# atsuki-ichikawa/KoeMorph

Hardware: AMD Instinct MI355X
Metric: blendshape frames/sec (52-coef, 256-win, d_model=256) (higher is better)
Workload: dtype f32; 1 GPU; C2: 256 windows/GPU x 136448 samples (8.5 s @16 kHz) -> 1024-pt STFT, hop 533, 80-bin log-mel (257 frames) -> dual-stream attention d_model=256, 8 heads, window 256 -> 52 coefficients + EMA; from audio resident in HBM (rotating batches); windows_per_gpu=256, samples_per_window=136448, parallelism=window-sharded x1, no collective

## Files before the change

### include/koemorph.h

```cpp
#ifndef KOEMORPH_H
#define KOEMORPH_H

#include <stdint.h>

#ifdef __cplusplus
extern "C" {
#endif

#define KM_ABI_VERSION 2

typedef enum km_status {
    KM_OK = 0,
    KM_ERR_INVALID_ARG = -1,
    KM_ERR_UNSUPPORTED = -2,
    KM_ERR_NOT_FINALIZED = -3,
    KM_ERR_WORKSPACE = -4,
    KM_ERR_HIP = -5,
    KM_ERR_NOT_READY = -6
} km_status;

typedef struct km_context* km_handle;

typedef enum km_mel_scale { KM_MEL_SLANEY = 0, KM_MEL_HTK = 1 } km_mel_scale;
typedef enum km_pad_mode { KM_PAD_CONSTANT = 0, KM_PAD_REFLECT = 1 } km_pad_mode;
// ... 228 lines not shown
                        void* stream);
int km_stream_step_attn(km_handle h, const float* emotion_dev, float* out_dev, uint8_t* fired_dev, uint8_t* ready_dev, int32_t* backlog_dev,
                        float* raw_dev, float* attn_dev, void* stream);

int km_legacy_stream_create(km_handle h, int64_t n_streams, int64_t buffer_samples, int64_t audio_length);
int km_legacy_stream_push(km_handle h, const float* samples_dev, int64_t n_per_stream, const int32_t* counts_dev, void* stream);
int km_legacy_stream_tick(km_handle h, float* out_dev, uint8_t* ready_dev, void* stream);
int km_legacy_stream_reset(km_handle h, void* stream);

int km_enable_stage_timing(km_handle h, int32_t enable);
int km_stage_times(km_handle h, float* ms3);

int km_egemaps_plan_create(void** plan_out);
int km_egemaps_plan_destroy(void* plan);
int64_t km_egemaps_num_frames(int64_t L);
int64_t km_egemaps_workspace_floats(int64_t B, int64_t L);
int km_egemaps_functionals(void* plan, const float* audio_dev, int64_t B, int64_t L, int32_t normalize, float* work_dev,
                           int64_t work_floats, float* out_dev, void* stream);
int km_egemaps_records(const float* work_dev, int64_t B, int64_t L, float* rec_host, void* stream);
int km_egemaps_track_from_records(float* rec_dev, int64_t B, int64_t nf, void* stream);
int km_egemaps_functionals_from_records(const float* rec_dev, int64_t B, int64_t nf, float* out_dev, void* stream);
int km_linear(const float* x_dev, const float* w_dev, const float* b_dev, int64_t B, int64_t K, int64_t N, float* out_dev, void* stream);
int km_gemm_kernel_choice(int64_t M, int64_t N, int64_t K, int64_t batch);

int km_emotion_stream_create(void** es, int64_t n_streams, double context_window_s, double update_interval_s, int64_t max_updates);
int km_emotion_stream_destroy(void* es);
int km_emotion_stream_set_compression(void* es, const float* w_dev, const float* b_dev, void* stream);
int km_emotion_stream_push(void* es, const float* samples_dev, int64_t n_per_stream, const int32_t* counts_dev, void* stream);
int km_emotion_stream_update(void* es, float* emotion_dev, uint8_t* valid_dev, uint8_t* updated_dev, void* stream);
int km_emotion_stream_reset_streams(void* es, const uint8_t* mask_dev, void* stream);
int km_emotion_stream_features(void* es, float* features_dev, float* slots_dev, void* stream);

int km_prosody_plan_create(void** plan_out);
int km_prosody_plan_destroy(void* plan);
int64_t km_prosody_num_frames(int64_t L);
int64_t km_prosody_workspace_floats(int64_t B, int64_t L);
int km_prosody_features(void* plan, const float* audio_dev, int64_t B, int64_t L, int64_t row_stride, float* work_dev, int64_t work_floats,
                        float* out_dev, float* frames_dev, void* stream);
int km_prosody_windows(void* plan, const float* clip_dev, int64_t clip_len, const int32_t* start_samples_dev, int64_t W, int64_t L,
                       float* work_dev, int64_t work_floats, float* out_dev, void* stream);
int km_emotion_stream_create_basic(void** es, int64_t n_streams, double context_window_s, double update_interval_s, int64_t max_updates);

int km_emotion_clip_create(void** ec, double context_window_s, double update_interval_s, int64_t max_slots);
int km_emotion_clip_destroy(void* ec);
int km_emotion_clip_set_compression(void* ec, const float* w_dev, const float* b_dev, void* stream);
int64_t km_emotion_clip_num_rows(void* ec, int64_t clip_len);
// ... 71 lines not shown
```

### koemorph_amd/_lib.py

```python
from __future__ import annotations

import ctypes as C
import os
from typing import Optional

from . import build as _build

KM_ABI_VERSION = 2


class KoeMorphError(RuntimeError):
    def __init__(self, code: int, msg: str):
        super().__init__(f"libkoemorph_hip: {msg} (status {code})")
        self.code = code


class KMMelConfig(C.Structure):
    _fields_ = [("sample_rate", C.c_int32), ("n_fft", C.c_int32), ("hop_length", C.c_int32),
                ("n_mels", C.c_int32), ("f_min", C.c_float), ("f_max", C.c_float),
                ("mel_scale", C.c_int32), ("slaney_norm", C.c_int32), ("pad_mode", C.c_int32),
                ("window_norm", C.c_int32), ("log_mode", C.c_int32), ("amin", C.c_float),
                ("top_db", C.c_float), ("db_add", C.c_float), ("db_scale", C.c_float),
                ("log_eps", C.c_float)]

# ... 161 lines not shown
    "km_metrics_destroy": (C.c_int, [_p]),
    "km_metrics_reset": (C.c_int, [_p, _p]),
    "km_metrics_update": (C.c_int, [_p, _p, _p, _p, _i64, _p]),
    "km_metrics_compute": (C.c_int, [_p, _p, _p]),
    "km_attn_stats_create": (C.c_int, [C.POINTER(_p), _i32, _i32, _i64]),
    "km_attn_stats_destroy": (C.c_int, [_p]),
    "km_attn_stats_shape": (C.c_int, [_p, C.POINTER(_i32), C.POINTER(_i32)]),
    "km_attn_stats_reset": (C.c_int, [_p, _p]),
    "km_attn_stats_update": (C.c_int, [_p, _p, _i64, _p]),
    "km_attn_stats_update_masked": (C.c_int, [_p, _p, _p, _i64, _p]),
    "km_attn_stats_compute": (C.c_int, [_p, _p, _p]),
    "km_attn_stats_streams_create": (C.c_int, [C.POINTER(_p), _i64, _i32, _i32]),
    "km_attn_stats_streams_destroy": (C.c_int, [_p]),
    "km_attn_stats_streams_update": (C.c_int, [_p, _p, _p, _p]),
    "km_attn_stats_streams_reset": (C.c_int, [_p, _p, _p]),
    "km_attn_stats_streams_compute": (C.c_int, [_p, _p, _p]),
    "km_loss_terms_create": (C.c_int, [C.POINTER(_p)]),
    "km_loss_terms_destroy": (C.c_int, [_p]),
    "km_loss_terms_reset": (C.c_int, [_p, _p]),
    "km_loss_terms_update": (C.c_int, [_p, C.POINTER(KMLossConfig), C.c_float, C.c_float, _p, _p, _i64, _p, _p]),
    "km_loss_terms_compute": (C.c_int, [_p, _p, _p]),
    "km_linear": (C.c_int, [_p, _p, _p, _i64, _i64, _i64, _p, _p]),
    "km_gemm_kernel_choice": (C.c_int, [_i64, _i64, _i64, _i64]),
    "km_emotion_stream_create": (C.c_int, [C.POINTER(_p), _i64, C.c_double, C.c_double, _i64]),
    "km_emotion_stream_destroy": (C.c_int, [_p]),
    "km_emotion_stream_set_compression": (C.c_int, [_p, _p, _p, _p]),
    "km_emotion_stream_push": (C.c_int, [_p, _p, _i64, _p, _p]),
    "km_emotion_stream_update": (C.c_int, [_p, _p, _p, _p, _p]),
    "km_emotion_stream_reset_streams": (C.c_int, [_p, _p, _p]),
    "km_emotion_stream_features": (C.c_int, [_p, _p, _p, _p]),
    "km_emotion_stream_create_basic": (C.c_int, [C.POINTER(_p), _i64, C.c_double, C.c_double, _i64]),
    "km_prosody_plan_create": (C.c_int, [C.POINTER(_p)]),
    "km_prosody_plan_destroy": (C.c_int, [_p]),
    "km_prosody_num_frames": (_i64, [_i64]),
    "km_prosody_workspace_floats": (_i64, [_i64, _i64]),
    "km_prosody_features": (C.c_int, [_p, _p, _i64, _i64, _i64, _p, _i64, _p, _p, _p]),
    "km_prosody_windows": (C.c_int, [_p, _p, _i64, _p, _i64, _i64, _p, _i64, _p, _p]),
    "km_emotion_clip_create": (C.c_int, [C.POINTER(_p), C.c_double, C.c_double, _i64]),
    "km_emotion_clip_create_basic": (C.c_int, [C.POINTER(_p), C.c_double, C.c_double, _i64]),
    "km_emotion_clip_width": (C.c_int, [_p]),
    "km_emotion_clip_destroy": (C.c_int, [_p]),
    "km_emotion_clip_set_compression": (C.c_int, [_p, _p, _p, _p]),
    "km_emotion_clip_num_rows": (_i64, [_p, _i64]),
    "km_emotion_clip_build": (C.c_int, [_p, _p, _i64, _p, _p, _p]),
    "km_emotion_clip_build_batch": (C.c_int, [_p, _p, _i64, _i64, _p, _p, _p]),
    "km_emotion_clip_rows": (C.c_int, [_p, _p, _i64, _i64, _p, _i64, _i64, _i64, _p, _p, _p]),
# ... 55 lines not shown
```

### koemorph_amd/csrc/km_api.hip

```cpp
#include <hip/hip_runtime.h>

#include <cstdlib>
#include <cstring>
#include <utility>
#include <vector>

#include "km_api_internal.h"
#include "km_context.h"
#include "km_device.h"
#include "km_gemm.h"

using namespace km;

extern "C" {


int km_finalize(km_handle h, void* stream) {
    if (!h) return fail(KM_ERR_INVALID_ARG, "NULL handle");
    Context* c = h;
    int ndev = 0;
    if (hipGetDeviceCount(&ndev) != hipSuccess || ndev == 0)
        return fail(KM_ERR_HIP, "no HIP device: libkoemorph_hip has no CPU fallback");
    HIP_TRY(hipGetDevice(&c->device));
    if (!c->host_finalized)
// ... 127 lines not shown
    if (!c->fused_ok) {
        if (B > c->ws.windows || !c->ws.generic) return fail(KM_ERR_WORKSPACE, "generic workspace missing or too small: call km_reserve after km_finalize");
        return launch_core_generic(c, mel_dev, B, T_in, mel_short_dev, z_dev, out_dev, raw_dev, attn_mel_dev, stream);
    }
    return launch_core_fused(c, mel_dev, B, T_in, mel_short_dev, z_dev, out_dev, raw_dev, attn_mel_dev, nullptr, 1, stream);
}

static GemmArgs linear_args(const float* x_dev, const float* w_dev, const float* b_dev, int64_t B, int64_t K, int64_t N, float* out_dev) {
    GemmArgs g{};
    g.alpha = 1.f; g.batch2 = 1; g.kb_count = 1;
    g.A = x_dev; g.a_rs = K; g.a_cs = 1; g.B = w_dev; g.b_rs = 1; g.b_cs = K; g.C = out_dev; g.c_rs = N;
    g.M = (int)B; g.N = (int)N; g.K = (int)K; g.bias = b_dev; g.bias_mode = b_dev ? 1 : 0;
    return g;
}

int km_linear(const float* x_dev, const float* w_dev, const float* b_dev, int64_t B, int64_t K, int64_t N, float* out_dev, void* stream) {
    if (!x_dev || !w_dev || !out_dev || B <= 0 || K <= 0 || N <= 0) return fail(KM_ERR_INVALID_ARG, "km_linear: bad argument");
    return launch_gemm(linear_args(x_dev, w_dev, b_dev, B, K, N, out_dev), 1, stream);
}

int km_gemm_kernel_choice(int64_t M, int64_t N, int64_t K, int64_t batch) {
    if (M <= 0 || N <= 0 || K <= 0 || batch <= 0 || M > INT32_MAX || N > INT32_MAX || K > INT32_MAX || batch > INT32_MAX) return -1;
    return gemm_kernel_choice(linear_args(nullptr, nullptr, nullptr, M, K, N, nullptr), (int)batch);
}

int km_audio_energy(const float* features_dev, int64_t B, int64_t T, int64_t D, float* energy_dev, void* stream) {
    if (!features_dev || !energy_dev || B <= 0 || T <= 0 || D <= 0) return fail(KM_ERR_INVALID_ARG, "km_audio_energy: bad argument");
    return launch_audio_energy(features_dev, B, T, D, energy_dev, stream);
}

int km_legacy_forward_mel(km_handle h, const float* mel_dev, int64_t B, int64_t T_mel, float* out_dev, void* stream) {
    if (int rc = need_ready(h)) return rc;
    Context* c = h;
    if (c->kind != 1) return fail(KM_ERR_INVALID_ARG, "not a legacy handle (km_legacy_create)");
    if (!mel_dev || !out_dev || B <= 0 || T_mel <= 0) return fail(KM_ERR_INVALID_ARG, "km_legacy_forward_mel: bad argument");
    if (B > c->ws.windows || T_mel > c->ws.frames || !c->ws.generic)
        return fail(KM_ERR_WORKSPACE, "workspace too small for %lld windows x %lld frames: call km_reserve",
                    (long long)B, (long long)T_mel);
    return launch_legacy(c, mel_dev, B, T_mel, out_dev, stream);
}

int km_koemorph_reserve(km_handle h, int64_t max_batch, int64_t max_frames) {
    if (int rc = need_ready(h)) return rc;
    Context* c = h;
    if (c->kind != 2) return fail(KM_ERR_INVALID_ARG, "not a KoeMorphModel handle (km_koemorph_create)");
    if (max_batch <= 0 || max_frames <= 0) return fail(KM_ERR_INVALID_ARG, "km_koemorph_reserve: bad argument");
// ... 278 lines not shown
```

### koemorph_amd/csrc/km_context.h

```cpp
#pragma once

#include <cstdint>
#include <map>
#include <string>
#include <vector>

#include "koemorph.h"
#include "km_devbuf.h"

namespace km {

constexpr int kNumMouth = 28;
constexpr int kNumExpr = 24;
extern const int kMouthIdx[kNumMouth];
extern const int kExprIdx[kNumExpr];

struct HostParam {
    std::vector<int64_t> shape;
    std::vector<float> data;
    bool loaded = false;
};

struct Packed {
    std::vector<float> host;
    DevBuf<float> dev;
};

constexpr int kMelRpWaves = 8;
constexpr int kMelRpGroups = 4;
constexpr int kMelRpRow = 580;

struct MelPlan {
    km_mel_config cfg{};
    int n_freq = 0;
    std::vector<float> window;
    std::vector<float> twiddle;
    std::vector<int32_t> fb_start;
    std::vector<int32_t> fb_count;
    std::vector<int32_t> fb_offset;
    std::vector<float> fb_weight;
    std::vector<int32_t> fbg_gid;
    std::vector<int32_t> fbg_desc;
    std::vector<float> fbg_weight;
    int fbg_extent = 0;
    DevBuf<float> d_window, d_twiddle;
    DevBuf<int32_t> d_fb_start, d_fb_count, d_fb_offset;
    DevBuf<float> d_fb_weight;
    DevBuf<int32_t> d_fbg_gid, d_fbg_desc;
    DevBuf<float> d_fbg_weight;
    bool uploaded = false;
};

struct Options {
    int core_split = 0;
    int seq_per_window = 0;
    int seq_assemble = 0;
    int clip_assemble = 0;
    int generic_staged = 0;
    int mel_two_frame = 0;
    int emotion_separate = 0;
    int no_ln_fusion = 0, no_db_fusion = 0, no_score_fusion = 0, no_out_fusion = 0, no_v_fusion = 0;
    int legacy_no_merge = 0;
    int no_core_merge = 0;
    int core128 = 0;
    int legacy_no_tail_fusion = 0;
    int legacy_no_enc_fusion = 0;
    int legacy_no_attn_fusion = 0;
    int kmm_no_fuse = 0;
    int train_no_split = 0;
    int train_split_min_k = 0;
    int train_alone_max = 0;
    int train_no_dy_split = 0;
    int train_ln_fuse_rows = 0;
    int train_no_ln_fuse = 0;
    int train_colsum_gemm = 0;
    int train_no_fe_pack = 0;
    int train_attn_regs = 0;
    int train_no_dma = 0;
    int train_op_per_launch = 0;
    int train_bm32_below = 0;
    int train_tail_groups = 0;
};
void options_from_env(Options& o);
// ... 248 lines not shown
bool core_takes_power(Context* c, bool with_attention);
int launch_core_power(Context* c, MelPlan* plan, int64_t B, int64_t n_frames, const float* zemo, float* out, void* stream, const CoreSrc& src);
int core_route(Context* c, bool with_attention);

struct SeqFrames {
    float* pow;
    unsigned* fmax;
    int64_t n_rows;
    int frame_mul;
};
struct MelPack { float* xt; int T, KP; };
struct MelSrc {
    const float* audio; int64_t B, L;
    int64_t clip_len, win_step, win0; int wins_per_clip;
    const int* ring_start; const unsigned char* ready;
};
inline MelSrc mel_windows(const float* audio, int64_t B, int64_t L) { return {audio, B, L, L, 0, 0, 1, nullptr, nullptr}; }
inline MelSrc mel_clip_windows(const float* clips, int64_t clip_len, int64_t B, int64_t L, int64_t win_step, int64_t win0, int wins_per_clip) {
    return {clips, B, L, clip_len, win_step, win0, wins_per_clip, nullptr, nullptr};
}
inline MelSrc mel_rings(Context* c, const unsigned char* gate = nullptr) {
    return {c->st.ring, c->st.n_streams, c->st.ring_len, c->st.ring_len, 0, 0, 1, c->st.ring_wptr, gate ? gate : c->st.ring_ready};
}
struct MelCarry { const float* emotion = nullptr; float* zemo = nullptr; const SeqFrames* seq = nullptr; const MelPack* pack = nullptr; };
inline MelCarry mel_emotion(const float* emotion, float* zemo) { return {emotion, zemo, nullptr, nullptr}; }
inline MelCarry mel_to_frames(const SeqFrames* seq) { return {nullptr, nullptr, seq, nullptr}; }
inline MelCarry mel_to_pack(const MelPack* pack) { return {nullptr, nullptr, nullptr, pack}; }
int launch_mel_power(Context* c, MelPlan* p, const MelSrc& src, void* stream, const MelCarry& carry = {});
bool mel_rp_ok(Context* c, MelPlan* p);
bool clip_frames_shared(Context* c, MelPlan* p);
bool mel_packs(Context* c, MelPlan* p, int64_t n_frames, int64_t T);
int launch_mel_clip_span(Context* c, MelPlan* p, const float* clip, int64_t clip_len, const int* start_frames, int64_t B,
                         int min_start, int64_t n_span, int T, float* span, float* edge, void* stream);
int launch_train_clip_pack(Context* c, MelPlan* p, const float* span, const float* edge, const int* start_frames, int64_t B,
                           int min_start, int64_t n_span, int T, int KP, float* xt, void* stream);
bool mel_fuses_emotion(Context* c, MelPlan* p);
int launch_mel_power_with_logits(Context* c, MelPlan* p, const MelSrc& src, const float* emotion, float* zemo, void* stream,
                                 hipEvent_t emo_done = nullptr);
int clear_stale_maxima(Context* c, void* stream);

struct SeqAssemble {
    const float* pow; const unsigned* fmax; const float* left; const unsigned* lmax; const float* right; const unsigned* rmax;
    int64_t total; int nfc, stride, n_per_clip, E, T;
};
int launch_seq_assemble(Context* c, const SeqAssemble& s, int64_t nw, int64_t win0, void* stream);
int launch_seq_zero_maxima(unsigned* fmax, int64_t n_fmax, unsigned* emax, int64_t n_emax, void* stream);
int ensure_chunk_counters(Context* c, int64_t windows, void* stream);

struct ClipPlan { int route, E; int64_t n_span, stft_frames; };
ClipPlan clip_plan(Context* c, int64_t B, int64_t min_start, int64_t max_start, int mode);
int launch_clip_images(Context* c, MelPlan* plan, const float* clip, int64_t clip_len, const int* start_frames, int64_t B, int min_start,
                       int64_t n_span, int E, void* stream);
int launch_clip_assemble(Context* c, const int* start_frames, int64_t B, int min_start, int64_t n_span, int E, void* stream);
int launch_clip_pack_edges(Context* c, MelPlan* p, const int* start_frames, int64_t B, int min_start, int64_t n_span, int E, int KP, float* xt,
                           void* stream);
int launch_ring_push(Context* c, const float* samples, int64_t n_per_stream, void* stream);

int launch_lfifo_push(Context* c, const float* samples, int64_t n_per_stream, const int* counts, void* stream);
int launch_lfifo_pop(Context* c, unsigned char* ready_out, void* stream);
// ... 13 lines not shown
```

### koemorph_amd/csrc/km_device.h

```cpp
#pragma once

#include <hip/hip_runtime.h>

#include "koemorph.h"

namespace km {

struct LogParams {
    int log_mode;
    float amin, top_db, db_add, db_scale, log_eps;
};

__device__ __forceinline__ float clamp_lo(float x, float lo) { return __builtin_amdgcn_fmed3f(x, lo, __builtin_inff()); }
__device__ __forceinline__ float db10(float s, float amin) {
    return 3.01029995663981195f * __builtin_amdgcn_logf(clamp_lo(s, amin));
}

__device__ __forceinline__ void log_window_consts(const LogParams& p, float ref, float& ref_db, float& floor_db) {
    ref_db = db10(ref, p.amin);
    floor_db = (db10(ref, p.amin) - ref_db) - p.top_db;
}

__device__ __forceinline__ float db_finish(const LogParams& p, float dbs, float ref_db, float floor_db) {
    float v = dbs - ref_db;
// ... 136 lines not shown
                acc = fmaf(x.y, w[u + 1], acc);
                acc = fmaf(x.z, w[u + 2], acc);
                acc = fmaf(x.w, w[u + 3], acc);
            }
            part[q * DH + m] = acc;
        }
    }
    __syncthreads();
    if (tid < 64) {
        float s = 0.f;
#pragma unroll
        for (int i = 0; i < 2; ++i) {
            const int mm = lane + 64 * i;
            float hsum = e.be2[mm];
#pragma unroll
            for (int q = 0; q < 8; ++q) hsum += part[q * DH + mm];
            s += fmaxf(hsum, 0.f) * e.w2[mm];
        }
#pragma unroll
        for (int o = 32; o > 0; o >>= 1) s += __shfl_xor(s, o);
        if (lane == 0) e.zemo[b] = s + e.b2[0];
    }
    __syncthreads();
}

struct EmoShape { int d = 0, DH = 0; };

__device__ __forceinline__ void emotion_layer_f4(const float* __restrict__ w, int K, int N, const float* x, float* part) {
    const int tid = threadIdx.x;
    const int tpr = N >> 2;
    const int G = 512 / tpr;
    const int c4 = tid & (tpr - 1), g = tid / tpr;
    const int kc = (K + G - 1) / G;
    const int k0 = g * kc, k1 = (k0 + kc) < K ? (k0 + kc) : K;
    float4 acc = make_float4(0.f, 0.f, 0.f, 0.f);
    const float* wp = w + 4 * c4;
    for (int k = k0; k < k1; k += 16) {
        float4 wv[16];
#pragma unroll
        for (int u = 0; u < 16; ++u) wv[u] = (k + u) < k1 ? *reinterpret_cast<const float4*>(wp + (size_t)(k + u) * N) : make_float4(0.f, 0.f, 0.f, 0.f);
#pragma unroll
        for (int u = 0; u < 16; ++u) {
            const float xv = (k + u) < k1 ? x[k + u] : 0.f;
            acc.x = fmaf(xv, wv[u].x, acc.x); acc.y = fmaf(xv, wv[u].y, acc.y);
            acc.z = fmaf(xv, wv[u].z, acc.z); acc.w = fmaf(xv, wv[u].w, acc.w);
        }
// ... 56 lines not shown
```

### koemorph_amd/csrc/km_host.cpp

```cpp
#include <cctype>
#include <cmath>
#include <cstdlib>
#include <cstdarg>
#include <cstdio>
#include <cstring>

#include "km_context.h"
#include "km_kmmf.h"

namespace km {

const int kMouthIdx[kNumMouth] = {14, 15, 16, 17, 18, 19, 20, 21, 22, 23, 24, 25, 26, 27,
                                  28, 29, 30, 31, 32, 33, 34, 35, 36, 37, 38, 39, 40, 51};
const int kExprIdx[kNumExpr] = {0, 1, 2, 3, 4, 5, 6, 7, 8, 9, 10, 11, 12, 13,
                                41, 42, 43, 44, 45, 46, 47, 48, 49, 50};

static thread_local char g_err[512] = "";

void set_error(const char* fmt, ...) {
    va_list ap;
    va_start(ap, fmt);
    vsnprintf(g_err, sizeof(g_err), fmt, ap);
    va_end(ap);
}
// ... 586 lines not shown

static bool same_cfg(const km_mel_config& a, const km_mel_config& b) { return std::memcmp(&a, &b, sizeof(a)) == 0; }

MelPlan* find_or_add_plan(Context* c, const km_mel_config& cfg) {
    for (MelPlan* p : c->mel_plans)
        if (same_cfg(p->cfg, cfg)) return p;
    MelPlan* p = build_mel_plan(cfg);
    c->mel_plans.push_back(p);
    return p;
}

}

using namespace km;

namespace km { const char* last_error(); }

namespace km {
namespace {
struct OptName { const char* name; int Options::*field; };
const OptName kOptNames[] = {
    {"core_split", &Options::core_split}, {"seq_per_window", &Options::seq_per_window}, {"seq_assemble", &Options::seq_assemble}, {"clip_assemble", &Options::clip_assemble},
    {"generic_staged", &Options::generic_staged}, {"mel_two_frame", &Options::mel_two_frame},
    {"emotion_separate", &Options::emotion_separate}, {"no_ln_fusion", &Options::no_ln_fusion},
    {"no_db_fusion", &Options::no_db_fusion}, {"no_score_fusion", &Options::no_score_fusion},
    {"no_out_fusion", &Options::no_out_fusion}, {"no_v_fusion", &Options::no_v_fusion}, {"no_core_merge", &Options::no_core_merge}, {"core128", &Options::core128}, {"legacy_no_merge", &Options::legacy_no_merge}, {"kmm_no_fuse", &Options::kmm_no_fuse}, {"legacy_no_attn_fusion", &Options::legacy_no_attn_fusion}, {"legacy_no_enc_fusion", &Options::legacy_no_enc_fusion}, {"legacy_no_tail_fusion", &Options::legacy_no_tail_fusion},
    {"train_no_split", &Options::train_no_split}, {"train_tail_groups", &Options::train_tail_groups}, {"train_bm32_below", &Options::train_bm32_below}, {"train_op_per_launch", &Options::train_op_per_launch}, {"train_split_min_k", &Options::train_split_min_k}, {"train_no_dma", &Options::train_no_dma}, {"train_attn_regs", &Options::train_attn_regs}, {"train_no_fe_pack", &Options::train_no_fe_pack}, {"train_colsum_gemm", &Options::train_colsum_gemm}, {"train_no_ln_fuse", &Options::train_no_ln_fuse}, {"train_ln_fuse_rows", &Options::train_ln_fuse_rows}, {"train_no_dy_split", &Options::train_no_dy_split}, {"train_alone_max", &Options::train_alone_max},
};
}

void options_from_env(Options& o) {
    for (const OptName& n : kOptNames) {
        std::string env = "KM_";
        for (const char* p = n.name; *p; ++p) env += (char)std::toupper((unsigned char)*p);
        if (const char* v = std::getenv(env.c_str())) o.*(n.field) = *v ? std::atoi(v) : 1;
    }
    if (std::getenv("KM_GENERIC_NO_LN_FUSION")) o.no_ln_fusion = 1;
    if (std::getenv("KM_GENERIC_NO_DB_FUSION")) o.no_db_fusion = 1;
    if (std::getenv("KM_GENERIC_NO_SCORE_FUSION")) o.no_score_fusion = 1;
    if (std::getenv("KM_GENERIC_NO_OUT_FUSION")) o.no_out_fusion = 1;
    if (std::getenv("KM_GENERIC_NO_V_FUSION")) o.no_v_fusion = 1;
}

int set_option(Context* c, const char* name, long long value) {
    for (const OptName& n : kOptNames)
        if (std::strcmp(n.name, name) == 0) {
            c->opt.*(n.field) = (int)value;
// ... 283 lines not shown
```

### koemorph_amd/csrc/km_mel.hip

```cpp
#include <hip/hip_runtime.h>

#include <cstdlib>

#include "km_context.h"
#include "km_device.h"

namespace km {


namespace mel {
constexpr int FPB = 16;
constexpr int WAVES = 4;
constexpr int FFT_BUF = 1152;
}

__device__ __forceinline__ float2 cadd(float2 a, float2 b) { return make_float2(a.x + b.x, a.y + b.y); }
__device__ __forceinline__ float2 csub(float2 a, float2 b) { return make_float2(a.x - b.x, a.y - b.y); }
__device__ __forceinline__ float2 cmul(float2 a, float2 b) {
    return make_float2(a.x * b.x - a.y * b.y, a.x * b.y + a.y * b.x);
}

template <int R>
__device__ __forceinline__ float2 twiddle_const(float2 d, int idx) {
    const int s = idx * (16 / R);
// ... 38 lines not shown
    int64_t clip_len, win_step;
    int64_t win0;
    int wins_per_clip;
    const int* ring_start;
    const unsigned char* ready;
    int n_frames;
    int hop;
    int pad_mode;
    int n_mels;
    const float* window;
    const float2* twiddle;
    const int* fb_start;
    const int* fb_count;
    const int* fb_offset;
    const float* fb_weight;
    int fb_nnz;
    const int* fbg_gid;
    const int* fbg_desc;
    const float* fbg_weight;
    int fbg_nw;
    float* melpow;
    unsigned* melmax;
    EmoArgs emo;
    int frame_mul;
    unsigned* frame_max;
    unsigned* chunk_ctr;
    float* pack_xt;
    int pack_T, pack_KP;
    float pack_amin;
    const int* tab_start;
    float* tab_edge;
    int tab_min, tab_T, tab_span_wgs;
};

template <int NFFT, bool RING>
__device__ __forceinline__ void load_pair(const MelArgs& a, const float* __restrict__ x, int64_t Lv, int rs, int fa,
                                          int lane, float2 (&z)[NFFT / 64]) {
    constexpr int R0 = NFFT / 64;
    if (fa >= a.n_frames) {
#pragma unroll
        for (int i = 0; i < R0; ++i) z[i] = make_float2(0.f, 0.f);
        return;
    }
    const int64_t p0 = (int64_t)fa * a.hop - NFFT / 2;
    const bool have_b = fa + 1 < a.n_frames;
    if constexpr (RING) {
// ... 182 lines not shown
            }
        }
        __syncthreads();
        const int nf_here = (a.n_frames - f0) < FPB ? (a.n_frames - f0) : FPB;
        float* dst = a.melpow + ((int64_t)b * a.n_frames + f0) * a.n_mels;
        for (int i = tid; i < nf_here * a.n_mels; i += 256) dst[i] = outs[i];
    }
#pragma unroll
    for (int o = 32; o > 0; o >>= 1) vmax = fmaxf(vmax, __shfl_xor(vmax, o));
    if (lane == 0) redmax[wave] = vmax;
    __syncthreads();
    if (tid == 0) {
        const float mx = fmaxf(fmaxf(redmax[0], redmax[1]), fmaxf(redmax[2], redmax[3]));
        atomicMax(a.melmax + b, __float_as_uint(mx));
    }
}

#ifndef KM_MEL_SKIP
#define KM_MEL_SKIP 0
#endif
#ifdef KM_MEL_STAMP
#define KM_ASM asm volatile
__device__ unsigned long long km_mel_stamps[1024 * 8 * 24];
#define KM_STAMP(i)                                                  \
    do {                                                             \
        const unsigned long long now_ = __builtin_readcyclecounter(); \
        st_acc[i] += (unsigned)(now_ - st_last);                     \
        st_last = now_;                                              \
    } while (0)
#else
#define KM_ASM asm
#define KM_STAMP(i) do {} while (0)
#endif
namespace melrp {
constexpr int WAVES = kMelRpWaves, NT = 64 * WAVES, FPB = 16, NC = 512, FFT_BUF = 576, NGW = kMelRpGroups;
constexpr int NFS = kMelRpRow;
static_assert(WAVES == 8 && NFS % 64 == 4 && NFS >= 528, "mel stage layout");

typedef float v2f __attribute__((ext_vector_type(2)));

#define KM_ADD(D, A, B) "v_pk_add_f32 %[" #D "], %[" #A "], %[" #B "]\n\t"
#define KM_SUB(D, A, B) "v_pk_add_f32 %[" #D "], %[" #A "], %[" #B "] neg_lo:[0,1] neg_hi:[0,1]\n\t"
#define KM_ADD_NI(D, A, B) "v_pk_add_f32 %[" #D "], %[" #A "], %[" #B "] op_sel:[0,1] op_sel_hi:[1,0] neg_hi:[0,1]\n\t"
#define KM_SUB_NI(D, A, B) "v_pk_add_f32 %[" #D "], %[" #A "], %[" #B "] op_sel:[0,1] op_sel_hi:[1,0] neg_lo:[0,1]\n\t"
#define KM_ROT3(D, S) "v_pk_add_f32 %[" #D "], %[" #S "], %[" #S "] op_sel:[1,0] op_sel_hi:[0,1] neg_lo:[0,1] neg_hi:[1,1]\n\t"
#define KM_CMUL1(T, A, W) "v_pk_mul_f32 %[" #T "], %[" #A "], %[" #W "] op_sel_hi:[0,1]\n\t"
// ... 284 lines not shown
    int m;
    if (slot & 1) m = frame < 8 ? frame + 4 : (frame < 12 ? frame + 8 : frame + 16);
    else m = frame < 4 ? frame : (frame < 8 ? frame + 8 : frame + 12);
    return 32 * (slot >> 1) + m;
}

template <bool RING, bool PACK = false, bool TAB = false>
__global__ __launch_bounds__(512, 4) void mel_power_rp_kernel(MelArgs a) {
    using namespace melrp;
    extern __shared__ __attribute__((aligned(16))) float smem[];
    float2* fbuf = reinterpret_cast<float2*>(smem);
    float* pw = smem + WAVES * FFT_BUF * 2;
    float* redmax = pw + FPB * NFS;
    int* sched = reinterpret_cast<int*>(redmax + WAVES);
    float* fbw = redmax + WAVES + 4;

#ifdef KM_MEL_STAMP
    const unsigned long long st_entry = __builtin_readcyclecounter(), st_entry_rt = __builtin_amdgcn_s_memrealtime();
#endif
    const int tid = threadIdx.x, lane = tid & 63;
    const int wave = __builtin_amdgcn_readfirstlane(tid >> 6);
#if KM_MEL_REMAP
    const unsigned lin_ = blockIdx.x + gridDim.x * blockIdx.y;
    const int b = TAB ? ((int)blockIdx.x < a.tab_span_wgs ? 0 : 1 + (int)blockIdx.x - a.tab_span_wgs) : (int)(lin_ % gridDim.y);
    const int bx = TAB ? (b == 0 ? (int)blockIdx.x : 0) : (int)(lin_ / gridDim.y);
#else
    const int b = blockIdx.y, bx = (int)blockIdx.x;
    static_assert(!TAB, "the clip-span launch is laid out for KM_MEL_REMAP");
#endif
    const unsigned gx = TAB ? (b == 0 ? (unsigned)a.tab_span_wgs : 1u) : gridDim.x;
    const int n_frames = TAB && b > 0 ? 2 : a.n_frames;
    const int64_t gw = a.win0 + b;
    const int64_t clip = TAB ? 0 : gw / a.wins_per_clip;
    int tab_f0 = 0;
    if constexpr (TAB) { tab_f0 = b == 0 ? a.tab_min : a.tab_start[b - 1]; tab_f0 = tab_f0 < 0 ? 0 : tab_f0; }
    const int64_t woff = TAB ? (int64_t)tab_f0 * a.hop : (gw - clip * a.wins_per_clip) * a.win_step;
    const int64_t Lw = TAB ? (int64_t)(b == 0 ? a.n_frames - 1 : a.tab_T) * a.hop : a.L;
    const float* x = a.audio + clip * a.clip_len + (TAB && woff >= a.clip_len ? 0 : woff);
    const int Lv = (int)((a.clip_len - woff) < Lw ? (a.clip_len - woff) : Lw);
    if (a.ready && !a.ready[b]) return;
    const int rs = RING ? a.ring_start[b] : -1;
    v2f* buf = reinterpret_cast<v2f*>(fbuf + wave * FFT_BUF);
    const int n_chunks = (n_frames + FPB - 1) / FPB;
    const unsigned rd2 = lds_offset(buf + (lane >> 3) * 72 + (lane & 7)), rd3 = lds_offset(buf + lane * 9);
    const unsigned wr3 = lds_offset(buf + fft_lane_k0(lane) * 9 + (lane & 7));
    const int cbin = fft_lane_bin(lane);

    v2f zn[8];
    bool zn_ok = false;
    const int fmul = TAB ? (b == 0 ? 1 : a.tab_T) : a.frame_mul;
    auto first_frame = [&]() {
        if (KM_MEL_SKIP & 8) {
#pragma unroll
            for (int i = 0; i < 8; ++i) zn[i] = v2f{0.001f * lane, 0.5f + i};
            zn_ok = true;
        } else if (bx * FPB + wave < n_frames) zn_ok = load_frame_rp_fast<RING>(x, Lv, rs, a.hop, (bx * FPB + wave) * fmul, lane, zn);
    };
    if (!PACK && !TAB && !(KM_MEL_SKIP & 16) && a.emo.emo && bx == (int)gx - 1) {
        if (a.emo.d == 256 && a.emo.DH == 128) emotion_window_d256(a.emo, gw, pw);
        else emotion_window_generic(a.emo, EmoShape{a.emo.d, a.emo.DH}, gw, pw);
        first_frame();
    } else {
        first_frame();
    }

    const unsigned ctr_last = (unsigned)n_chunks - 1u;
    for (int i = tid; i < a.fbg_nw; i += NT) fbw[i] = a.fbg_weight[i];
    for (int i = tid; i < FPB * (NFS - 513); i += NT) pw[(i / (NFS - 513)) * NFS + 513 + i % (NFS - 513)] = 0.f;

    const int n2 = lane & 7, k0 = fft_lane_k0(lane);
    v2f win2[8], tw1[8], tw2[8], twp[4];
#pragma unroll
    for (int i = 0; i < 8; ++i) {
        win2[i] = v2f{a.window[2 * (lane + 64 * i)], a.window[2 * (lane + 64 * i) + 1]};
        tw1[i] = ld2(a.twiddle + ((2 * lane * bitrev(i, 3)) & 1023));
        tw2[i] = ld2(a.twiddle + ((16 * n2 * bitrev(i, 3)) & 1023));
    }
#pragma unroll
    for (int i = 0; i < 4; ++i) twp[i] = ld2(a.twiddle + cbin + 64 * i);

    int my_gid[NGW];
// ... 371 lines not shown

bool mel_packs(Context* c, MelPlan* p, int64_t n_frames, int64_t T) {
    const km_mel_config& m = p->cfg;
    return mel_rp_ok(c, p) && m.log_mode == KM_LOG_DB_MAX && m.top_db == m.db_add && m.db_scale > 0.f && n_frames >= T && n_frames >= 3;
}

static void mel_plan_args(MelPlan* p, MelArgs& a) {
    const km_mel_config& m = p->cfg;
    a.hop = m.hop_length; a.pad_mode = m.pad_mode;
    a.n_mels = m.n_mels; a.window = p->d_window; a.twiddle = reinterpret_cast<const float2*>(p->d_twiddle.p);
    a.fb_start = p->d_fb_start; a.fb_count = p->d_fb_count; a.fb_offset = p->d_fb_offset; a.fb_weight = p->d_fb_weight;
    a.fb_nnz = (int)p->fb_weight.size();
    a.fbg_gid = p->d_fbg_gid; a.fbg_desc = p->d_fbg_desc; a.fbg_weight = p->d_fbg_weight; a.fbg_nw = (int)p->fbg_weight.size();
}

int clear_stale_maxima(Context* c, void* stream) {
    if (c->melmax_dirty) {
        HIP_TRY(hipMemsetAsync(c->ws.melmax, 0, (size_t)c->ws.windows * sizeof(unsigned), (hipStream_t)stream));
        c->melmax_dirty = false;
    }
    return KM_OK;
}

int launch_mel_power_with_logits(Context* c, MelPlan* p, const MelSrc& src, const float* emotion, float* zemo, void* stream, hipEvent_t emo_done) {
    const bool rider = mel_fuses_emotion(c, p);
    if (!rider)
        if (int rc = launch_emotion(c, emotion, src.B, zemo, stream)) return rc;
    if (emo_done) HIP_TRY(hipEventRecord(emo_done, (hipStream_t)stream));
    return launch_mel_power(c, p, src, stream, rider ? mel_emotion(emotion, zemo) : MelCarry{});
}

int launch_mel_power(Context* c, MelPlan* p, const MelSrc& src, void* stream, const MelCarry& carry) {
    const km_mel_config& m = p->cfg;
    const SeqFrames* seq = carry.seq;
    const int64_t B = src.B, L = src.L;
    const int64_t n_frames = seq ? seq->n_rows : 1 + L / m.hop_length;
    if (m.pad_mode == KM_PAD_REFLECT && L <= m.n_fft / 2)
        return fail(KM_ERR_INVALID_ARG, "reflect padding needs more than n_fft/2 = %d samples (got %lld)", m.n_fft / 2, (long long)L);
    if (!seq && (B > c->ws.windows || n_frames > c->ws.frames))
        return fail(KM_ERR_WORKSPACE, "workspace holds %lld windows x %lld frames, need %lld x %lld: call km_reserve",
                    (long long)c->ws.windows, (long long)c->ws.frames, (long long)B, (long long)n_frames);
    if (!seq && m.n_mels > c->ws.mels)
        return fail(KM_ERR_WORKSPACE, "workspace rows hold %d mel bins, this plan has %d: call km_reserve", c->ws.mels, m.n_mels);
    const bool ring = src.ring_start != nullptr, plain = !ring && src.wins_per_clip <= 1;
    if ((carry.emotion != nullptr) + (seq != nullptr) + (carry.pack != nullptr) > 1 || (seq && !(mel_rp_ok(c, p) && !ring)) ||
        (carry.pack && !(plain && mel_packs(c, p, n_frames, carry.pack->T) && carry.pack->KP >= carry.pack->T + 3)) ||
        (carry.emotion && !(mel_fuses_emotion(c, p) && carry.zemo && src.wins_per_clip <= 1)))
        return fail(KM_ERR_UNSUPPORTED, "launch_mel_power: emotion rider, frame image or packed output requested for an unsupported configuration");
    if (!p->uploaded) return fail(KM_ERR_NOT_FINALIZED, "mel plan not uploaded (km_finalize / km_reserve first)");
    static PerDeviceOnce once;
    if (once.first(c->device)) {
        const struct { const void* fn; int lds; } kernels[] = {
            {(const void*)&mel_power_kernel<1024, false>, (int)mel_lds_bytes(1024)}, {(const void*)&mel_power_kernel<512, false>, (int)mel_lds_bytes(512)},
            {(const void*)&mel_power_kernel<1024, true>, (int)mel_lds_bytes(1024)}, {(const void*)&mel_power_kernel<512, true>, (int)mel_lds_bytes(512)},
            {(const void*)&mel_power_rp_kernel<false>, 160 * 1024}, {(const void*)&mel_power_rp_kernel<true>, 160 * 1024},
            {(const void*)&mel_power_rp_kernel<false, true>, 160 * 1024}};
        for (const auto& k : kernels) HIP_TRY(hipFuncSetAttribute(k.fn, hipFuncAttributeMaxDynamicSharedMemorySize, k.lds));
    }
    hipStream_t st = (hipStream_t)stream;
    if (int rc = ensure_chunk_counters(c, B, stream)) return rc;
    if (!seq)
        if (int rc = clear_stale_maxima(c, stream)) return rc;
    MelArgs a;
    mel_plan_args(p, a);
    a.audio = src.audio; a.L = L; a.clip_len = src.clip_len; a.win_step = src.win_step; a.win0 = src.win0;
    a.wins_per_clip = src.wins_per_clip > 0 ? src.wins_per_clip : 1; a.n_frames = (int)n_frames;
    a.ring_start = src.ring_start; a.ready = src.ready;
    a.melpow = c->ws.melpow; a.melmax = c->ws.melmax;
    a.frame_mul = 1; a.frame_max = nullptr; a.chunk_ctr = c->ws_chunkctr;
    a.pack_xt = nullptr; a.pack_T = a.pack_KP = 0; a.pack_amin = m.amin;
    a.tab_start = nullptr; a.tab_edge = nullptr; a.tab_min = a.tab_T = a.tab_span_wgs = 0;
    if (carry.pack) { a.pack_xt = carry.pack->xt; a.pack_T = carry.pack->T; a.pack_KP = carry.pack->KP; }
    if (seq) { a.melpow = seq->pow; a.frame_max = seq->fmax; a.frame_mul = seq->frame_mul; a.melmax = nullptr; }
    if (carry.emotion) {
        auto dvp = [&](const char* name) { return (const float*)c->packed.at(name).dev; };
        a.emo.emo = carry.emotion; a.emo.ED = c->ED; a.emo.zemo = carry.zemo;
        a.emo.d = c->d; a.emo.DH = c->DH;
        a.emo.wee_t = (c->d == 256 && c->DH == 128) ? dvp("wee_t256") : dvp("wee_t"); a.emo.bee = dvp("bee"); a.emo.lg = dvp("eln_g"); a.emo.lb = dvp("eln_b");
        a.emo.we2 = dvp("we2"); a.emo.be2 = dvp("be2"); a.emo.w2 = dvp("w2"); a.emo.b2 = dvp("b2");
    }
    const int n_chunks = (int)((n_frames + mel::FPB - 1) / mel::FPB);
    int per_window = (int)((512 + B / 2) / B);
    if (per_window > n_chunks) per_window = n_chunks;
    if (per_window < 1) per_window = 1;
    const dim3 grid((unsigned)per_window, (unsigned)B);
    if (mel_rp_ok(c, p)) {
        const size_t ldsrp = melrp_lds_bytes(a.fbg_nw);
        if (carry.pack) hipLaunchKernelGGL((mel_power_rp_kernel<false, true>), grid, dim3(melrp::NT), ldsrp, st, a);
        else if (!ring) hipLaunchKernelGGL((mel_power_rp_kernel<false>), grid, dim3(melrp::NT), ldsrp, st, a);
        else hipLaunchKernelGGL((mel_power_rp_kernel<true>), grid, dim3(melrp::NT), ldsrp, st, a);
        HIP_TRY(hipGetLastError());
        return KM_OK;
    }
    const size_t lds = mel_lds_bytes(m.n_fft, m.n_mels, a.fb_nnz);
    if (m.n_fft == 1024 && !ring) hipLaunchKernelGGL((mel_power_kernel<1024, false>), grid, dim3(256), lds, st, a);
    else if (m.n_fft == 1024) hipLaunchKernelGGL((mel_power_kernel<1024, true>), grid, dim3(256), lds, st, a);
    else if (!ring) hipLaunchKernelGGL((mel_power_kernel<512, false>), grid, dim3(256), lds, st, a);
    else hipLaunchKernelGGL((mel_power_kernel<512, true>), grid, dim3(256), lds, st, a);
    HIP_TRY(hipGetLastError());
    return KM_OK;
}

struct ClipPackArgs {
    const float* span;
    int edge_off;
    const int* start;
    int min_start, n_span, T, KP, n_mels, row_stride, tile_cols;
    float amin;
// ... 168 lines not shown
        int w = w0 + hop;
        w -= w >= ring_len ? ring_len : 0;
        wptr[s] = w;
        const int f = frames[s] + 1;
        frames[s] = f;
        if ((int64_t)f * hop >= ring_len) ready[s] = 1;
    }
}

int launch_ring_push(Context* c, const float* samples, int64_t n_per_stream, void* stream) {
    hipLaunchKernelGGL(ring_push_kernel, dim3((unsigned)c->st.n_streams), dim3(256), 0, (hipStream_t)stream, c->st.ring,
                       c->st.ring_wptr, c->st.ring_frames, c->st.ring_ready, samples, (int)n_per_stream, c->st.ring_hop,
                       (int)c->st.ring_len);
    HIP_TRY(hipGetLastError());
    return KM_OK;
}

LogParams plan_log_params(MelPlan* p) { return log_params(p->cfg); }

#ifdef KM_MEL_STAMP
extern "C" __attribute__((visibility("default"))) int km_debug_mel_stamps(unsigned long long* out, int n) {
    return (int)hipMemcpyFromSymbol(out, HIP_SYMBOL(km_mel_stamps), (size_t)n * sizeof(unsigned long long));
}
#endif

}
```

Before: 1.881 million frames/s.

## Compute emotion logits in dedicated grouped workgroups instead of riding mel blocks

```diff
diff --git a/include/koemorph.h b/include/koemorph.h
--- a/include/koemorph.h
+++ b/include/koemorph.h
@@ -274,6 +274,7 @@
 int km_egemaps_functionals_from_records(const float* rec_dev, int64_t B, int64_t nf, float* out_dev, void* stream);
 int km_linear(const float* x_dev, const float* w_dev, const float* b_dev, int64_t B, int64_t K, int64_t N, float* out_dev, void* stream);
 int km_gemm_kernel_choice(int64_t M, int64_t N, int64_t K, int64_t batch);
+int km_mel_role_table(int64_t windows, int32_t per_window, int32_t group, int64_t n_ids, int32_t* out);
 
 int km_emotion_stream_create(void** es, int64_t n_streams, double context_window_s, double update_interval_s, int64_t max_updates);
 int km_emotion_stream_destroy(void* es);
diff --git a/koemorph_amd/_lib.py b/koemorph_amd/_lib.py
--- a/koemorph_amd/_lib.py
+++ b/koemorph_amd/_lib.py
@@ -207,6 +207,7 @@
     "km_loss_terms_compute": (C.c_int, [_p, _p, _p]),
     "km_linear": (C.c_int, [_p, _p, _p, _i64, _i64, _i64, _p, _p]),
     "km_gemm_kernel_choice": (C.c_int, [_i64, _i64, _i64, _i64]),
+    "km_mel_role_table": (C.c_int, [_i64, _i32, _i32, _i64, _p]),
     "km_emotion_stream_create": (C.c_int, [C.POINTER(_p), _i64, C.c_double, C.c_double, _i64]),
     "km_emotion_stream_destroy": (C.c_int, [_p]),
     "km_emotion_stream_set_compression": (C.c_int, [_p, _p, _p, _p]),
diff --git a/koemorph_amd/csrc/km_api.hip b/koemorph_amd/csrc/km_api.hip
--- a/koemorph_amd/csrc/km_api.hip
+++ b/koemorph_amd/csrc/km_api.hip
@@ -173,6 +173,10 @@
 int km_gemm_kernel_choice(int64_t M, int64_t N, int64_t K, int64_t batch) {
     if (M <= 0 || N <= 0 || K <= 0 || batch <= 0 || M > INT32_MAX || N > INT32_MAX || K > INT32_MAX || batch > INT32_MAX) return -1;
     return gemm_kernel_choice(linear_args(nullptr, nullptr, nullptr, M, K, N, nullptr), (int)batch);
+}
+
+int km_mel_role_table(int64_t windows, int32_t per_window, int32_t group, int64_t n_ids, int32_t* out) {
+    return mel_role_table(windows, per_window, group, n_ids, out);
 }
 
 int km_audio_energy(const float* features_dev, int64_t B, int64_t T, int64_t D, float* energy_dev, void* stream) {
diff --git a/koemorph_amd/csrc/km_context.h b/koemorph_amd/csrc/km_context.h
--- a/koemorph_amd/csrc/km_context.h
+++ b/koemorph_amd/csrc/km_context.h
@@ -26,8 +26,12 @@
     DevBuf<float> dev;
 };
 
+#ifndef KM_EMO_GROUP
+#define KM_EMO_GROUP 2
+#endif
 constexpr int kMelRpWaves = 8;
 constexpr int kMelRpGroups = 4;
+constexpr int kMelEmoGroup = KM_EMO_GROUP;
 constexpr int kMelRpRow = 580;
 
 struct MelPlan {
@@ -59,6 +63,7 @@
     int generic_staged = 0;
     int mel_two_frame = 0;
     int emotion_separate = 0;
+    int emotion_rider = 0;
     int no_ln_fusion = 0, no_db_fusion = 0, no_score_fusion = 0, no_out_fusion = 0, no_v_fusion = 0;
     int legacy_no_merge = 0;
     int no_core_merge = 0;
@@ -353,10 +358,10 @@
 inline MelSrc mel_rings(Context* c, const unsigned char* gate = nullptr) {
     return {c->st.ring, c->st.n_streams, c->st.ring_len, c->st.ring_len, 0, 0, 1, c->st.ring_wptr, gate ? gate : c->st.ring_ready};
 }
-struct MelCarry { const float* emotion = nullptr; float* zemo = nullptr; const SeqFrames* seq = nullptr; const MelPack* pack = nullptr; };
-inline MelCarry mel_emotion(const float* emotion, float* zemo) { return {emotion, zemo, nullptr, nullptr}; }
-inline MelCarry mel_to_frames(const SeqFrames* seq) { return {nullptr, nullptr, seq, nullptr}; }
-inline MelCarry mel_to_pack(const MelPack* pack) { return {nullptr, nullptr, nullptr, pack}; }
+struct MelCarry { const float* emotion = nullptr; float* zemo = nullptr; const SeqFrames* seq = nullptr; const MelPack* pack = nullptr; int emo_group = 0; };
+inline MelCarry mel_emotion(const float* emotion, float* zemo, int emo_group = 0) { return {emotion, zemo, nullptr, nullptr, emo_group}; }
+inline MelCarry mel_to_frames(const SeqFrames* seq) { return {nullptr, nullptr, seq, nullptr, 0}; }
+inline MelCarry mel_to_pack(const MelPack* pack) { return {nullptr, nullptr, nullptr, pack, 0}; }
 int launch_mel_power(Context* c, MelPlan* p, const MelSrc& src, void* stream, const MelCarry& carry = {});
 bool mel_rp_ok(Context* c, MelPlan* p);
 bool clip_frames_shared(Context* c, MelPlan* p);
@@ -366,6 +371,8 @@
 int launch_train_clip_pack(Context* c, MelPlan* p, const float* span, const float* edge, const int* start_frames, int64_t B,
                            int min_start, int64_t n_span, int T, int KP, float* xt, void* stream);
 bool mel_fuses_emotion(Context* c, MelPlan* p);
+bool mel_emotion_grouped(Context* c, MelPlan* p);
+int mel_role_table(int64_t windows, int per_window, int group, int64_t n_ids, int32_t* out);
 int launch_mel_power_with_logits(Context* c, MelPlan* p, const MelSrc& src, const float* emotion, float* zemo, void* stream,
                                  hipEvent_t emo_done = nullptr);
 int clear_stale_maxima(Context* c, void* stream);
diff --git a/koemorph_amd/csrc/km_device.h b/koemorph_amd/csrc/km_device.h
--- a/koemorph_amd/csrc/km_device.h
+++ b/koemorph_amd/csrc/km_device.h
@@ -182,6 +182,136 @@
         if (lane == 0) e.zemo[b] = s + e.b2[0];
     }
     __syncthreads();
+}
+
+template <int G>
+__device__ __forceinline__ void emotion_group_d256(const EmoArgs& e, int64_t win0, int b0, int ng, const unsigned char* ready, float* scratch) {
+    constexpr int d = 256, DH = 128, WS = 1536;
+    const int tid = threadIdx.x, lane = tid & 63;
+    const int wave = __builtin_amdgcn_readfirstlane(tid >> 6);
+    const int n = tid & 255, h1 = __builtin_amdgcn_readfirstlane(tid >> 8);
+    const int m = tid & 127, h2 = tid >> 7;
+    const float bee_n = e.bee[n];
+    float lg[4], lb[4], be2v[2], w2v[2];
+#pragma unroll
+    for (int i = 0; i < 4; ++i) { lg[i] = e.lg[lane + 64 * i]; lb[i] = e.lb[lane + 64 * i]; }
+#pragma unroll
+    for (int i = 0; i < 2; ++i) { be2v[i] = e.be2[lane + 64 * i]; w2v[i] = e.w2[lane + 64 * i]; }
+    const float b2 = e.b2[0];
+    auto load1 = [&](int q, float (&w)[64]) {
+        const float* wp = e.wee_t + (size_t)64 * q * d + n;
+#pragma unroll
+        for (int u = 0; u < 64; ++u) w[u] = wp[u * d];
+    };
+    auto run1 = [&](int q, const float (&w)[64]) {
+#pragma unroll 1
+        for (int g = 0; g < ng; ++g) {
+            const float* emo_s = scratch + g * WS;
+            float acc = 0.f;
+#pragma unroll
+            for (int u = 0; u < 64; u += 4) {
+                const float4 x = *reinterpret_cast<const float4*>(emo_s + 64 * q + u);
+                acc = fmaf(x.x, w[u], acc);
+                acc = fmaf(x.y, w[u + 1], acc);
+                acc = fmaf(x.z, w[u + 2], acc);
+                acc = fmaf(x.w, w[u + 3], acc);
+            }
+            scratch[g * WS + 512 + q * d + n] = acc;
+        }
+    };
+    auto load2 = [&](int q, float (&w)[32]) {
+        const float* wp = e.we2 + (size_t)32 * q * DH + m;
+#pragma unroll
+        for (int u = 0; u < 32; ++u) w[u] = wp[u * DH];
+    };
+    auto run2 = [&](int q, const float (&w)[32]) {
+#pragma unroll 1
+        for (int g = 0; g < ng; ++g) {
+            const float* e1 = scratch + g * WS + 256;
+            float acc = 0.f;
+#pragma unroll
+            for (int u = 0; u < 32; u += 4) {
+                const float4 x = *reinterpret_cast<const float4*>(e1 + 32 * q + u);
+                acc = fmaf(x.x, w[u], acc);
+                acc = fmaf(x.y, w[u + 1], acc);
+                acc = fmaf(x.z, w[u + 2], acc);
+                acc = fmaf(x.w, w[u + 3], acc);
+            }
+            scratch[g * WS + 512 + q * DH + m] = acc;
+        }
+    };
+    {
+        float w[64];
+        load1(2 * h1, w);
+        for (int i = tid; i < ng * d; i += 512) {
+            const int g = i >> 8, k = i & 255;
+            scratch[g * WS + k] = k < e.ED ? e.emo[(win0 + b0 + g) * e.ED + k] : 0.f;
+        }
+        __syncthreads();
+        run1(2 * h1, w);
+        load1(2 * h1 + 1, w);
+        run1(2 * h1 + 1, w);
+    }
+    float w2r[32];
+    load2(2 * h2, w2r);
+    __syncthreads();
+    for (int i = tid; i < ng * d; i += 512) {
+        const int g = i >> 8;
+        const float* part = scratch + g * WS + 512;
+        float s = bee_n;
+#pragma unroll
+        for (int q = 0; q < 4; ++q) s += part[q * d + n];
+        scratch[g * WS + 256 + n] = s;
+    }
+    __syncthreads();
+    for (int g = wave; g < ng; g += 8) {
+        float* e1 = scratch + g * WS + 256;
+        float x[4], s = 0.f;
+#pragma unroll
+        for (int i = 0; i < 4; ++i) { x[i] = e1[lane + 64 * i]; s += x[i]; }
+#pragma unroll
+        for (int o = 32; o > 0; o >>= 1) s += __shfl_xor(s, o);
+        const float mean = s * (1.0f / d);
+        float v = 0.f;
+#pragma unroll
+        for (int i = 0; i < 4; ++i) { const float t = x[i] - mean; v += t * t; }
+#pragma unroll
+        for (int o = 32; o > 0; o >>= 1) v += __shfl_xor(v, o);
+        const float rstd = 1.0f / sqrtf(v * (1.0f / d) + 1e-5f);
+#pragma unroll
+        for (int i = 0; i < 4; ++i) {
+            const int c = lane + 64 * i;
+            e1[c] = (x[i] - mean) * rstd * lg[i] + lb[i];
+        }
+    }
+    __syncthreads();
+    run2(2 * h2, w2r);
+    load2(2 * h2 + 1, w2r);
+    run2(2 * h2 + 1, w2r);
+    __syncthreads();
+    for (int g = wave; g < ng; g += 8) {
+        const float* part = scratch + g * WS + 512;
+        float s = 0.f;
+#pragma unroll
+        for (int i = 0; i < 2; ++i) {
+            const int mm = lane + 64 * i;
+            float hsum = be2v[i];
+#pragma unroll
+            for (int q = 0; q < 8; ++q) hsum += part[q * DH + mm];
+            s += fmaxf(hsum, 0.f) * w2v[i];
+        }
+#pragma unroll
+        for (int o = 32; o > 0; o >>= 1) s += __shfl_xor(s, o);
+        if (lane == 0 && (!ready || ready[b0 + g])) e.zemo[win0 + b0 + g] = s + b2;
+    }
+}
+
+struct MelRole { int kind, b, bx; };
+__host__ __device__ inline MelRole mel_role(unsigned lin, int windows, int per_window, int groups) {
+    if (lin < (unsigned)groups) return {1, (int)lin, 0};
+    const unsigned r = lin - (unsigned)groups;
+    if (r >= (unsigned)windows * (unsigned)per_window) return {0, 0, 0};
+    return {2, (int)(r % (unsigned)windows), (int)(r / (unsigned)windows)};
 }
 
 struct EmoShape { int d = 0, DH = 0; };
diff --git a/koemorph_amd/csrc/km_host.cpp b/koemorph_amd/csrc/km_host.cpp
--- a/koemorph_amd/csrc/km_host.cpp
+++ b/koemorph_amd/csrc/km_host.cpp
@@ -632,7 +632,7 @@
 const OptName kOptNames[] = {
     {"core_split", &Options::core_split}, {"seq_per_window", &Options::seq_per_window}, {"seq_assemble", &Options::seq_assemble}, {"clip_assemble", &Options::clip_assemble},
     {"generic_staged", &Options::generic_staged}, {"mel_two_frame", &Options::mel_two_frame},
-    {"emotion_separate", &Options::emotion_separate}, {"no_ln_fusion", &Options::no_ln_fusion},
+    {"emotion_separate", &Options::emotion_separate}, {"emotion_rider", &Options::emotion_rider}, {"no_ln_fusion", &Options::no_ln_fusion},
     {"no_db_fusion", &Options::no_db_fusion}, {"no_score_fusion", &Options::no_score_fusion},
     {"no_out_fusion", &Options::no_out_fusion}, {"no_v_fusion", &Options::no_v_fusion}, {"no_core_merge", &Options::no_core_merge}, {"core128", &Options::core128}, {"legacy_no_merge", &Options::legacy_no_merge}, {"kmm_no_fuse", &Options::kmm_no_fuse}, {"legacy_no_attn_fusion", &Options::legacy_no_attn_fusion}, {"legacy_no_enc_fusion", &Options::legacy_no_enc_fusion}, {"legacy_no_tail_fusion", &Options::legacy_no_tail_fusion},
     {"train_no_split", &Options::train_no_split}, {"train_tail_groups", &Options::train_tail_groups}, {"train_bm32_below", &Options::train_bm32_below}, {"train_op_per_launch", &Options::train_op_per_launch}, {"train_split_min_k", &Options::train_split_min_k}, {"train_no_dma", &Options::train_no_dma}, {"train_attn_regs", &Options::train_attn_regs}, {"train_no_fe_pack", &Options::train_no_fe_pack}, {"train_colsum_gemm", &Options::train_colsum_gemm}, {"train_no_ln_fuse", &Options::train_no_ln_fuse}, {"train_ln_fuse_rows", &Options::train_ln_fuse_rows}, {"train_no_dy_split", &Options::train_no_dy_split}, {"train_alone_max", &Options::train_alone_max},
diff --git a/koemorph_amd/csrc/km_mel.hip b/koemorph_amd/csrc/km_mel.hip
--- a/koemorph_amd/csrc/km_mel.hip
+++ b/koemorph_amd/csrc/km_mel.hip
@@ -84,6 +84,7 @@
     float* melpow;
     unsigned* melmax;
     EmoArgs emo;
+    int n_windows, emo_groups;
     int frame_mul;
     unsigned* frame_max;
     unsigned* chunk_ctr;
@@ -312,6 +313,7 @@
 #ifdef KM_MEL_STAMP
 #define KM_ASM asm volatile
 __device__ unsigned long long km_mel_stamps[1024 * 8 * 24];
+__device__ unsigned long long km_mel_group_stamps[2 * 128];
 #define KM_STAMP(i)                                                  \
     do {                                                             \
         const unsigned long long now_ = __builtin_readcyclecounter(); \
@@ -642,8 +644,28 @@
     const int wave = __builtin_amdgcn_readfirstlane(tid >> 6);
 #if KM_MEL_REMAP
     const unsigned lin_ = blockIdx.x + gridDim.x * blockIdx.y;
-    const int b = TAB ? ((int)blockIdx.x < a.tab_span_wgs ? 0 : 1 + (int)blockIdx.x - a.tab_span_wgs) : (int)(lin_ % gridDim.y);
-    const int bx = TAB ? (b == 0 ? (int)blockIdx.x : 0) : (int)(lin_ / gridDim.y);
+    const MelRole role = TAB ? MelRole{2, 0, 0} : mel_role(lin_, a.n_windows, (int)gridDim.x, PACK ? 0 : a.emo_groups);
+    if (!TAB && role.kind == 0) return;
+    if constexpr (!PACK && !TAB) {
+        if (role.kind == 1) {
+            static_assert(kMelEmoGroup * 1536 <= WAVES * FFT_BUF * 2 + FPB * NFS, "the group scratch has to fit the launch's dynamic LDS");
+#ifdef KM_MEL_STAMP
+            const unsigned long long g_rt0 = __builtin_amdgcn_s_memrealtime();
+#endif
+            const int g0 = role.b * kMelEmoGroup;
+            const int ng = a.n_windows - g0 < kMelEmoGroup ? a.n_windows - g0 : kMelEmoGroup;
+            if (!(KM_MEL_SKIP & 16)) emotion_group_d256<kMelEmoGroup>(a.emo, a.win0, g0, ng, a.ready, smem);
+#ifdef KM_MEL_STAMP
+            if (tid == 0 && role.b < 128) {
+                km_mel_group_stamps[2 * role.b] = g_rt0;
+                km_mel_group_stamps[2 * role.b + 1] = __builtin_amdgcn_s_memrealtime();
+            }
+#endif
+            return;
+        }
+    }
+    const int b = TAB ? ((int)blockIdx.x < a.tab_span_wgs ? 0 : 1 + (int)blockIdx.x - a.tab_span_wgs) : role.b;
+    const int bx = TAB ? (b == 0 ? (int)blockIdx.x : 0) : role.bx;
 #else
     const int b = blockIdx.y, bx = (int)blockIdx.x;
     static_assert(!TAB, "the clip-span launch is laid out for KM_MEL_REMAP");
@@ -676,7 +698,7 @@
             zn_ok = true;
         } else if (bx * FPB + wave < n_frames) zn_ok = load_frame_rp_fast<RING>(x, Lv, rs, a.hop, (bx * FPB + wave) * fmul, lane, zn);
     };
-    if (!PACK && !TAB && !(KM_MEL_SKIP & 16) && a.emo.emo && bx == (int)gx - 1) {
+    if (!PACK && !TAB && !(KM_MEL_SKIP & 16) && a.emo.emo && a.emo_groups == 0 && bx == (int)gx - 1) {
         if (a.emo.d == 256 && a.emo.DH == 128) emotion_window_d256(a.emo, gw, pw);
         else emotion_window_generic(a.emo, EmoShape{a.emo.d, a.emo.DH}, gw, pw);
         first_frame();
@@ -1094,12 +1116,27 @@
     return KM_OK;
 }
 
+bool mel_emotion_grouped(Context* c, MelPlan* p) {
+    return KM_MEL_REMAP && mel_fuses_emotion(c, p) && c->d == 256 && c->DH == 128 && !c->opt.emotion_rider;
+}
+
 int launch_mel_power_with_logits(Context* c, MelPlan* p, const MelSrc& src, const float* emotion, float* zemo, void* stream, hipEvent_t emo_done) {
-    const bool rider = mel_fuses_emotion(c, p);
-    if (!rider)
+    const bool fused = mel_fuses_emotion(c, p);
+    if (!fused)
         if (int rc = launch_emotion(c, emotion, src.B, zemo, stream)) return rc;
     if (emo_done) HIP_TRY(hipEventRecord(emo_done, (hipStream_t)stream));
-    return launch_mel_power(c, p, src, stream, rider ? mel_emotion(emotion, zemo) : MelCarry{});
+    return launch_mel_power(c, p, src, stream, fused ? mel_emotion(emotion, zemo, mel_emotion_grouped(c, p) ? kMelEmoGroup : 0) : MelCarry{});
+}
+
+int mel_role_table(int64_t windows, int per_window, int group, int64_t n_ids, int32_t* out) {
+    if (windows <= 0 || windows > 65535 || per_window <= 0 || per_window > 512 || group < 0 || n_ids < 0 || !out)
+        return fail(KM_ERR_INVALID_ARG, "mel_role_table: bad argument");
+    const int groups = group > 0 ? (int)((windows + group - 1) / group) : 0;
+    for (int64_t i = 0; i < n_ids; ++i) {
+        const MelRole r = mel_role((unsigned)i, (int)windows, per_window, groups);
+        out[3 * i] = r.kind; out[3 * i + 1] = r.b; out[3 * i + 2] = r.bx;
+    }
+    return KM_OK;
 }
 
 int launch_mel_power(Context* c, MelPlan* p, const MelSrc& src, void* stream, const MelCarry& carry) {
@@ -1117,8 +1154,9 @@
     const bool ring = src.ring_start != nullptr, plain = !ring && src.wins_per_clip <= 1;
     if ((carry.emotion != nullptr) + (seq != nullptr) + (carry.pack != nullptr) > 1 || (seq && !(mel_rp_ok(c, p) && !ring)) ||
         (carry.pack && !(plain && mel_packs(c, p, n_frames, carry.pack->T) && carry.pack->KP >= carry.pack->T + 3)) ||
-        (carry.emotion && !(mel_fuses_emotion(c, p) && carry.zemo && src.wins_per_clip <= 1)))
-        return fail(KM_ERR_UNSUPPORTED, "launch_mel_power: emotion rider, frame image or packed output requested for an unsupported configuration");
+        (carry.emotion && !(mel_fuses_emotion(c, p) && carry.zemo && src.wins_per_clip <= 1)) ||
+        (carry.emo_group && !(carry.emotion && carry.emo_group == kMelEmoGroup && KM_MEL_REMAP && c->d == 256 && c->DH == 128)))
+        return fail(KM_ERR_UNSUPPORTED, "launch_mel_power: emotion logits (rider or groups), frame image or packed output requested for an unsupported configuration");
     if (!p->uploaded) return fail(KM_ERR_NOT_FINALIZED, "mel plan not uploaded (km_finalize / km_reserve first)");
     static PerDeviceOnce once;
     if (once.first(c->device)) {
@@ -1140,6 +1178,7 @@
     a.ring_start = src.ring_start; a.ready = src.ready;
     a.melpow = c->ws.melpow; a.melmax = c->ws.melmax;
     a.frame_mul = 1; a.frame_max = nullptr; a.chunk_ctr = c->ws_chunkctr;
+    a.n_windows = (int)B; a.emo_groups = carry.emo_group ? (int)((B + carry.emo_group - 1) / carry.emo_group) : 0;
     a.pack_xt = nullptr; a.pack_T = a.pack_KP = 0; a.pack_amin = m.amin;
     a.tab_start = nullptr; a.tab_edge = nullptr; a.tab_min = a.tab_T = a.tab_span_wgs = 0;
     if (carry.pack) { a.pack_xt = carry.pack->xt; a.pack_T = carry.pack->T; a.pack_KP = carry.pack->KP; }
@@ -1155,7 +1194,7 @@
     int per_window = (int)((512 + B / 2) / B);
     if (per_window > n_chunks) per_window = n_chunks;
     if (per_window < 1) per_window = 1;
-    const dim3 grid((unsigned)per_window, (unsigned)B);
+    const dim3 grid((unsigned)per_window, (unsigned)(B + (a.emo_groups + per_window - 1) / per_window));
     if (mel_rp_ok(c, p)) {
         const size_t ldsrp = melrp_lds_bytes(a.fbg_nw);
         if (carry.pack) hipLaunchKernelGGL((mel_power_rp_kernel<false, true>), grid, dim3(melrp::NT), ldsrp, st, a);
@@ -1370,6 +1409,9 @@
 extern "C" __attribute__((visibility("default"))) int km_debug_mel_stamps(unsigned long long* out, int n) {
     return (int)hipMemcpyFromSymbol(out, HIP_SYMBOL(km_mel_stamps), (size_t)n * sizeof(unsigned long long));
 }
-#endif
-
-}
+extern "C" __attribute__((visibility("default"))) int km_debug_mel_group_stamps(unsigned long long* out, int n) {
+    return (int)hipMemcpyFromSymbol(out, HIP_SYMBOL(km_mel_group_stamps), (size_t)n * sizeof(unsigned long long));
+}
+#endif
+
+}
```

Measured after the change: 1.927 million frames/s (median of 6 runs). 2.5% higher.
